# Chris10M/Ev2Hands

Measured on AMD Instinct MI355X. Metric: event-windows/sec at B=256 N=2048 (f16x2), higher is better.
Workload: dtype f32 (each f32 operand split into 2 fp16 planes with per-window power-of-two range scaling, 3 plane products per MAC on the f16 MFMA, f32 accumulate); 1 GPU; TEHNet.forward+MANO both hands, B=256/GPU N=2048 C=4 fp32, E-clouds, random-init 342-key checkpoint, synthetic MANO-shaped assets; global_batch=256, points=2048, channels=4, precision=f16x2, forwards_in_flight=1, world_size_seen=1, parallelism=batch-shard x1

## Files before the change

ev2hands_amd/csrc/points.hip:

```cpp
#include <cstdlib>
#include "common.hpp"
#include "ev2hands_hip.h"

namespace {

typedef float f32x2 __attribute__((ext_vector_type(2)));

__device__ __forceinline__ float sqnorm3(float x, float y, float z) {
    return __fadd_rn(__fadd_rn(__fmul_rn(x, x), __fmul_rn(y, y)), __fmul_rn(z, z));
}

__global__ __launch_bounds__(256) void prep_points_kernel(float* __restrict__ xyz_cm, int C, int N, int mhlnes,
                                                          float4* __restrict__ pts4, float4* __restrict__ feat8,
                                                          unsigned* __restrict__ amax) {
    const int b = blockIdx.y;
    const int n = blockIdx.x * 256 + threadIdx.x;
    float* base = xyz_cm + (size_t)b * C * N;
    float f[8];
#pragma unroll
    for (int c = 0; c < 8; ++c) f[c] = (c < C && n < N) ? base[(size_t)c * N + n] : 0.f;
    if (mhlnes && n < N) {
        float s = f[3];
        for (int c = 4; c < C; ++c) s = __fadd_rn(s, f[c]);
        s = s / (float)(C - 3);
        f[2] = s;
        base[(size_t)2 * N + n] = s;
    }
    if (amax) {
        unsigned m = 0u;
#pragma unroll
        for (int c = 0; c < 8; ++c) m = max(m, __float_as_uint(f[c]) & 0x7fffffffu);
        m = wave_max_u32_dpp(m);
        if ((threadIdx.x & 63) == 0 && m) atomicMax(&amax[b], m);
    }
    if (n >= N) return;
    pts4[(size_t)b * N + n] = make_float4(f[0], f[1], f[2], sqnorm3(f[0], f[1], f[2]));
    feat8[((size_t)b * N + n) * 2 + 0] = make_float4(f[0], f[1], f[2], f[3]);
    feat8[((size_t)b * N + n) * 2 + 1] = make_float4(f[4], f[5], f[6], f[7]);
}

struct FpsJobs {
    int njobs;
    int S[3];
    const int64_t* init[3];
    int32_t* idx[3];
    float4* ctr[3];
    int s_begin, s_end;
    float* state; int state_ld;
};

template <int PPT, int THREADS = 256, bool LDS_PTS = true>
__global__ __launch_bounds__(THREADS) void fps_kernel(const float4* __restrict__ pts4, int N, FpsJobs jobs) {
    extern __shared__ __attribute__((aligned(16))) char smem_raw[];
    float4* spts = reinterpret_cast<float4*>(smem_raw);
    constexpr int NW = THREADS / 64;
    __shared__ unsigned long long skey[2][NW];

    const int b = blockIdx.x;
    const int job = blockIdx.y;
    const int S = jobs.S[job];
    const int tid = threadIdx.x, lane = tid & 63, wave = tid >> 6;
    const float4* src = pts4 + (size_t)b * N;

    constexpr bool REG_PTS = !(PPT >= 32 && THREADS >= 1024);
    float px[REG_PTS ? PPT : 1], py[REG_PTS ? PPT : 1], pz[REG_PTS ? PPT : 1], md[PPT];
#pragma unroll
    for (int j = 0; j < PPT; ++j) {
        const int p = j * THREADS + tid;
        if constexpr (REG_PTS || LDS_PTS) {
            float4 v = (p < N) ? src[p] : make_float4(0.f, 0.f, 0.f, 0.f);
            if (LDS_PTS && p < N) spts[p] = v;
            if constexpr (REG_PTS) { px[j] = v.x; py[j] = v.y; pz[j] = v.z; }
        }
        md[j] = 1e10f;
    }
    __syncthreads();
    int tid_v = tid;
    auto coord = [&](int j, float& x, float& y, float& z) {
        if constexpr (REG_PTS) { x = px[j]; y = py[j]; z = pz[j]; }
        else {
            const unsigned pc = (unsigned)min(j * THREADS + tid_v, N - 1);
            const float4 v = *reinterpret_cast<const float4*>(reinterpret_cast<const char*>(src) + (size_t)pc * sizeof(float4));
            x = v.x; y = v.y; z = v.z;
        }
    };

    int far = (int)jobs.init[job][b];
    int32_t* oidx = jobs.idx[job] + (size_t)b * S;
    float4* octr = jobs.ctr[job] + (size_t)b * S;
    const int i_begin = min(jobs.s_begin, S), i_end = min(jobs.s_end, S);
    if (i_begin >= i_end) return;
    float* st = jobs.state ? jobs.state + ((size_t)b * jobs.njobs + job) * jobs.state_ld : nullptr;
    if (i_begin > 0) {
#pragma unroll
        for (int j = 0; j < PPT; ++j) md[j] = st[j * THREADS + tid];
        far = reinterpret_cast<const int*>(st)[jobs.state_ld - 4];
    }

    for (int i = i_begin; i < i_end; ++i) {
        if constexpr (!REG_PTS) asm volatile("" : "+v"(tid_v));
        const float4 c = LDS_PTS ? spts[far] : src[far];
        if (tid == 0) { oidx[i] = far; octr[i] = c; }
        unsigned long long best = 0ull;
        if constexpr (PPT >= 2) {
            const f32x2 cx = {c.x, c.x}, cy = {c.y, c.y}, cz = {c.z, c.z};
#pragma unroll
            for (int j = 0; j < PPT; j += 2) {
                float x0, y0, z0, x1, y1, z1;
                coord(j, x0, y0, z0);
                coord(j + 1, x1, y1, z1);
                const f32x2 dx = f32x2{x0, x1} - cx, dy = f32x2{y0, y1} - cy, dz = f32x2{z0, z1} - cz;
                const f32x2 d = (dx * dx + dy * dy) + dz * dz;
#pragma unroll
                for (int e = 0; e < 2; ++e) {
                    const int p = (j + e) * THREADS + tid;
                    if (d[e] < md[j + e]) md[j + e] = d[e];
                    const unsigned long long key =
                        ((unsigned long long)__float_as_uint(md[j + e]) << 32) | (unsigned long long)(0xffffffffu - (unsigned)p);
                    if (p < N && key > best) best = key;
                }
                if constexpr (!REG_PTS) {
                    if ((j & 6) == 6) __builtin_amdgcn_sched_barrier(0);
                }
            }
        } else {
#pragma unroll
            for (int j = 0; j < PPT; ++j) {
                const int p = j * THREADS + tid;
                float x0, y0, z0;
                coord(j, x0, y0, z0);
                const float dx = __fsub_rn(x0, c.x), dy = __fsub_rn(y0, c.y), dz = __fsub_rn(z0, c.z);
                const float d = sqnorm3(dx, dy, dz);
                if (d < md[j]) md[j] = d;
                const unsigned long long key =
                    ((unsigned long long)__float_as_uint(md[j]) << 32) | (unsigned long long)(0xffffffffu - (unsigned)p);
                if (p < N && key > best) best = key;
            }
        }
        best = wave_max_u64_dpp(best);
        if (lane == 0) skey[i & 1][wave] = best;
        __syncthreads();
        unsigned long long k0 = skey[i & 1][0];
#pragma unroll
        for (int w = 1; w < NW; ++w) { const unsigned long long kw = skey[i & 1][w]; k0 = k0 > kw ? k0 : kw; }
        far = (int)(0xffffffffu - (unsigned)(k0 & 0xffffffffull));
    }
    if (i_end < S) {
#pragma unroll
        for (int j = 0; j < PPT; ++j) st[j * THREADS + tid] = md[j];
        if (tid == 0) reinterpret_cast<int*>(st)[jobs.state_ld - 4] = far;
    }
}

struct BallArgs {
    int nrad;
    float r2[3];
    int K[3];
    int32_t* gidx[3];
    int32_t* cnt;
    int cpw;
    int nchunk;
    int s_off, s_cnt;
};

constexpr int BALL_CTR_PER_WG = 4, BALL_UNR = 4;

__global__ __launch_bounds__(256) void ball_query_kernel(const float4* __restrict__ pts4, const float4* __restrict__ ctr4,
                                                         int N, int S, BallArgs a) {
    const int L = xcd_remap(blockIdx.x, gridDim.x);
    const int b = L / a.nchunk;
    const int tid = threadIdx.x, lane = tid & 63, wave = tid >> 6;
    const float4* src = pts4 + (size_t)b * N;
    (void)tid;
    const int s_begin = a.s_off + (L - b * a.nchunk) * a.cpw;
    for (int s = s_begin + wave; s < s_begin + a.cpw && s < a.s_off + a.s_cnt; s += 4) {
        const float4 c = ctr4[(size_t)b * S + s];
        int cnt[3] = {0, 0, 0};
        int first[3] = {0, 0, 0};
        int32_t* gbase[3];
#pragma unroll
        for (int i = 0; i < 3; ++i) gbase[i] = (i < a.nrad) ? a.gidx[i] + ((size_t)b * S + s) * a.K[i] : nullptr;
        for (int base = 0; base < N; base += 64 * BALL_UNR) {
            float d[BALL_UNR];
#pragma unroll
            for (int u = 0; u < BALL_UNR; ++u) {
                const int p = base + 64 * u + lane;
                const float4 q = src[p < N ? p : N - 1];
                const float dot = __fmaf_rn(c.z, q.z, __fmaf_rn(c.y, q.y, __fmul_rn(c.x, q.x)));
                d[u] = __fadd_rn(__fadd_rn(__fmul_rn(-2.f, dot), c.w), q.w);
            }
            bool done = true;
#pragma unroll
            for (int i = 0; i < 3; ++i) {
                if (i < a.nrad && cnt[i] < a.K[i]) {
#pragma unroll
                    for (int u = 0; u < BALL_UNR; ++u) {
                        const int p = base + 64 * u + lane;
                        const bool in = (p < N) && !(d[u] > a.r2[i]);
                        const unsigned long long m = __ballot(in);
                        if (cnt[i] == 0 && m != 0ull) first[i] = base + 64 * u + __ffsll((long long)m) - 1;
                        const int pos = cnt[i] + (int)__builtin_amdgcn_mbcnt_hi((unsigned)(m >> 32), __builtin_amdgcn_mbcnt_lo((unsigned)m, 0u));
                        if (in && pos < a.K[i]) gbase[i][pos] = p;
                        cnt[i] += __popcll(m);
                    }
                    done = done && (cnt[i] >= a.K[i]);
                }
            }
            if (done) break;
        }
#pragma unroll
        for (int i = 0; i < 3; ++i) {
            if (i < a.nrad) {
                const int have = cnt[i] < a.K[i] ? cnt[i] : a.K[i];
                for (int pos = have + lane; pos < a.K[i]; pos += 64)
                    a.gidx[i][((size_t)b * S + s) * a.K[i] + pos] = first[i];
                if (a.cnt && lane == 0) a.cnt[((size_t)b * S + s) * a.nrad + i] = have;
            }
        }
    }
}

constexpr int NN_PTS_PER_WG = 256;
constexpr int NN_MAX_N2 = 4096;

__global__ __launch_bounds__(256) void three_nn_interp_kernel(const float4* __restrict__ pts1, const float4* __restrict__ pts2,
                                                              int N1, int N2, const float* __restrict__ feat2, int ldf2, int D,
                                                              float* __restrict__ out, int ldo,
                                                              int32_t* __restrict__ nn_idx, float* __restrict__ nn_w,
                                                              unsigned* __restrict__ amax, int ppw) {
    extern __shared__ __attribute__((aligned(16))) char smem_raw[];
    float4* s2 = reinterpret_cast<float4*>(smem_raw);
    int* sidx = reinterpret_cast<int*>(s2 + N2);
    float* sw = reinterpret_cast<float*>(sidx + NN_PTS_PER_WG * 3);
    const int b = blockIdx.y;
    const int tid = threadIdx.x, lane = tid & 63, wave = tid >> 6;
    for (int p = tid; p < N2; p += 256) s2[p] = pts2[(size_t)b * N2 + p];
    __syncthreads();

    const int n = blockIdx.x * ppw + tid;
    if (tid < ppw && n < N1) {
        const float4 q = pts1[(size_t)b * N1 + n];
        float d0 = INFINITY, d1 = INFINITY, d2 = INFINITY;
        int i0 = 0, i1 = 0, i2 = 0;
        for (int s = 0; s < N2; ++s) {
            const float4 c = s2[s];
            const float dot = __fmaf_rn(q.z, c.z, __fmaf_rn(q.y, c.y, __fmul_rn(q.x, c.x)));
            const float d = __fadd_rn(__fadd_rn(__fmul_rn(-2.f, dot), q.w), c.w);
            if (d < d2) {
                if (d < d1) {
                    d2 = d1; i2 = i1;
                    if (d < d0) { d1 = d0; i1 = i0; d0 = d; i0 = s; }
                    else        { d1 = d;  i1 = s; }
                } else { d2 = d; i2 = s; }
            }
        }
        const float r0 = __fdiv_rn(1.0f, __fadd_rn(d0, 1e-8f));
        const float r1 = __fdiv_rn(1.0f, __fadd_rn(d1, 1e-8f));
        const float r2 = __fdiv_rn(1.0f, __fadd_rn(d2, 1e-8f));
        const float norm = __fadd_rn(__fadd_rn(r0, r1), r2);
        const float w0 = __fdiv_rn(r0, norm), w1 = __fdiv_rn(r1, norm), w2 = __fdiv_rn(r2, norm);
        sidx[tid * 3 + 0] = i0; sidx[tid * 3 + 1] = i1; sidx[tid * 3 + 2] = i2;
        sw[tid * 3 + 0] = w0; sw[tid * 3 + 1] = w1; sw[tid * 3 + 2] = w2;
        if (nn_idx) {
            int32_t* o = nn_idx + ((size_t)b * N1 + n) * 3;
            o[0] = i0; o[1] = i1; o[2] = i2;
        }
        if (nn_w) {
            float* o = nn_w + ((size_t)b * N1 + n) * 3;
            o[0] = w0; o[1] = w1; o[2] = w2;
        }
    }
    __syncthreads();
    if (!out) return;
    const int D4 = D >> 2;
    float am = 0.f;
    const int pw = ppw >> 2;
#pragma unroll 1
    for (int t0 = wave * pw; t0 < wave * pw + pw; t0 += 4) {
        if (blockIdx.x * ppw + t0 >= N1) break;
        for (int c = lane; c < D4; c += 64) {
            float4 a[4], bq[4], cq[4];
            float w0[4], w1[4], w2[4];
#pragma unroll
            for (int u = 0; u < 4; ++u) {
                const int t = t0 + u;
                const int j0 = sidx[t * 3 + 0], j1 = sidx[t * 3 + 1], j2 = sidx[t * 3 + 2];
                w0[u] = sw[t * 3 + 0]; w1[u] = sw[t * 3 + 1]; w2[u] = sw[t * 3 + 2];
                const bool live = blockIdx.x * ppw + t < N1;
                a[u] = reinterpret_cast<const float4*>(feat2 + ((size_t)b * N2 + (live ? j0 : 0)) * ldf2)[c];
                bq[u] = reinterpret_cast<const float4*>(feat2 + ((size_t)b * N2 + (live ? j1 : 0)) * ldf2)[c];
                cq[u] = reinterpret_cast<const float4*>(feat2 + ((size_t)b * N2 + (live ? j2 : 0)) * ldf2)[c];
            }
#pragma unroll
            for (int u = 0; u < 4; ++u) {
                const int nn = blockIdx.x * ppw + t0 + u;
                if (nn >= N1) break;
                float4 r;
                r.x = __fadd_rn(__fadd_rn(__fmul_rn(a[u].x, w0[u]), __fmul_rn(bq[u].x, w1[u])), __fmul_rn(cq[u].x, w2[u]));
                r.y = __fadd_rn(__fadd_rn(__fmul_rn(a[u].y, w0[u]), __fmul_rn(bq[u].y, w1[u])), __fmul_rn(cq[u].y, w2[u]));
                r.z = __fadd_rn(__fadd_rn(__fmul_rn(a[u].z, w0[u]), __fmul_rn(bq[u].z, w1[u])), __fmul_rn(cq[u].z, w2[u]));
                r.w = __fadd_rn(__fadd_rn(__fmul_rn(a[u].w, w0[u]), __fmul_rn(bq[u].w, w1[u])), __fmul_rn(cq[u].w, w2[u]));
                reinterpret_cast<float4*>(out + ((size_t)b * N1 + nn) * ldo)[c] = r;
                am = fmaxf(fmaxf(am, fmaxf(fabsf(r.x), fabsf(r.y))), fmaxf(fabsf(r.z), fabsf(r.w)));
            }
        }
    }
    if (amax) {
        const unsigned m = wave_max_u32_dpp(__float_as_uint(am));
        if (lane == 0 && m) atomicMax(&amax[b], m);
    }
}

}

extern "C" int ev2h_prep_points(float* xyz_cm, int B, int C, int N, int mhlnes, float* pts4, float* feat8, uint32_t* amax,
                                ev2h_stream_t stream) {
    EV2H_CHECK_ARG(xyz_cm && pts4 && feat8);
    EV2H_CHECK_ARG(B > 0 && N > 0 && C >= 4 && C <= 8);
    dim3 grid(ceil_div(N, 256), B);
    prep_points_kernel<<<grid, 256, 0, (hipStream_t)stream>>>(xyz_cm, C, N, mhlnes, (float4*)pts4, (float4*)feat8, amax);
    EV2H_CHECK_LAUNCH();
    return EV2H_OK;
}

size_t ev2h_fps_state_ld(int N) {
    const int threads = N <= 2048 ? 256 : (N <= 8192 ? 512 : 1024);
    const int ppt = N <= 256 ? 1 : N <= 512 ? 2 : N <= 1024 ? 4 : N <= 2048 ? 8 : N <= 4096 ? 8 : N <= 8192 ? 16 : N <= 16384 ? 16 : 32;
    return (size_t)threads * ppt + 4;
}

int ev2h_fps_multi_chunk(const float* pts4, int B, int N, int njobs, const int* S, const int64_t* const* init, int32_t* const* idx, float* const* ctr4,
                         int s_begin, int s_end, float* state, ev2h_stream_t stream);

extern "C" int ev2h_fps_multi(const float* pts4, int B, int N, int njobs, const int* S, const int64_t* const* init,
                              int32_t* const* idx, float* const* ctr4, ev2h_stream_t stream) {
    return ev2h_fps_multi_chunk(pts4, B, N, njobs, S, init, idx, ctr4, 0, 0x7fffffff, nullptr, stream);
}

int ev2h_fps_multi_chunk(const float* pts4, int B, int N, int njobs, const int* S, const int64_t* const* init, int32_t* const* idx, float* const* ctr4,
                         int s_begin, int s_end, float* state, ev2h_stream_t stream) {
    EV2H_CHECK_ARG(pts4 && S && init && idx && ctr4);
    EV2H_CHECK_ARG(B > 0 && N > 0 && N <= 32768 && njobs >= 1 && njobs <= 3);
    EV2H_CHECK_ARG(s_begin >= 0 && s_end > s_begin);
    FpsJobs jobs{};
    jobs.njobs = njobs;
    jobs.s_begin = s_begin; jobs.s_end = s_end; jobs.state = state; jobs.state_ld = (int)ev2h_fps_state_ld(N);
    for (int j = 0; j < njobs; ++j) {
        EV2H_CHECK_ARG(S[j] > 0 && init[j] && idx[j] && ctr4[j]);
        jobs.S[j] = S[j];
        jobs.init[j] = init[j];
        jobs.idx[j] = idx[j];
        jobs.ctr[j] = (float4*)ctr4[j];
        EV2H_CHECK_ARG(state || (s_begin == 0 && s_end >= S[j]));
    }
    dim3 grid(B, njobs);
    const size_t lds = (size_t)N * sizeof(float4);
    hipStream_t st = (hipStream_t)stream;
    const float4* p = (const float4*)pts4;
    if (N > 2048 && N <= 8192) {
        static PerDevice attr_set{};
        EV2H_ONCE_PER_DEVICE(attr_set,
            EV2H_CHECK_HIP(hipFuncSetAttribute(reinterpret_cast<const void*>(fps_kernel<8, 512, true>),
                                               hipFuncAttributeMaxDynamicSharedMemorySize, 4096 * 16));
            EV2H_CHECK_HIP(hipFuncSetAttribute(reinterpret_cast<const void*>(fps_kernel<16, 512, true>),
                                               hipFuncAttributeMaxDynamicSharedMemorySize, 8192 * 16)););
    }
    if (N <= 256) fps_kernel<1><<<grid, 256, lds, st>>>(p, N, jobs);
    else if (N <= 512) fps_kernel<2><<<grid, 256, lds, st>>>(p, N, jobs);
    else if (N <= 1024) fps_kernel<4><<<grid, 256, lds, st>>>(p, N, jobs);
    else if (N <= 2048) fps_kernel<8><<<grid, 256, lds, st>>>(p, N, jobs);
    else if (N <= 4096) fps_kernel<8, 512, true><<<grid, 512, lds, st>>>(p, N, jobs);
    else if (N <= 8192) fps_kernel<16, 512, true><<<grid, 512, lds, st>>>(p, N, jobs);
    else if (N <= 16384) fps_kernel<16, 1024, false><<<grid, 1024, 0, st>>>(p, N, jobs);
    else fps_kernel<32, 1024, false><<<grid, 1024, 0, st>>>(p, N, jobs);
    EV2H_CHECK_LAUNCH();
    return EV2H_OK;
}

extern "C" int ev2h_fps(const float* pts4, int B, int N, int S, const int64_t* init, int32_t* idx, float* ctr4,
                        ev2h_stream_t stream) {
    return ev2h_fps_multi(pts4, B, N, 1, &S, &init, &idx, &ctr4, stream);
}

int ev2h_ball_query_range(const float* pts4, const float* ctr4, int B, int N, int S, int s_off, int s_cnt, int nrad, const double* radius,
                          const int* nsample, int32_t* const* gidx, int32_t* cnt, ev2h_stream_t stream);

extern "C" int ev2h_ball_query(const float* pts4, const float* ctr4, int B, int N, int S, int nrad, const double* radius,
                               const int* nsample, int32_t* const* gidx, int32_t* cnt, ev2h_stream_t stream) {
    return ev2h_ball_query_range(pts4, ctr4, B, N, S, 0, S, nrad, radius, nsample, gidx, cnt, stream);
}

int ev2h_ball_query_range(const float* pts4, const float* ctr4, int B, int N, int S, int s_off, int s_cnt, int nrad, const double* radius,
                          const int* nsample, int32_t* const* gidx, int32_t* cnt, ev2h_stream_t stream) {
    EV2H_CHECK_ARG(pts4 && ctr4 && radius && nsample && gidx);
    EV2H_CHECK_ARG(B > 0 && N > 0 && N <= 32768 && S > 0 && nrad >= 1 && nrad <= 3 && s_off >= 0 && s_cnt > 0 && s_off + s_cnt <= S);
    BallArgs a{};
    a.nrad = nrad;
    for (int i = 0; i < nrad; ++i) {
        EV2H_CHECK_ARG(gidx[i] && nsample[i] > 0);
        a.r2[i] = (float)(radius[i] * radius[i]);
        a.K[i] = nsample[i];
        a.gidx[i] = gidx[i];
    }
    a.cnt = cnt;
    a.cpw = BALL_CTR_PER_WG;
    a.s_off = s_off; a.s_cnt = s_cnt;
    a.nchunk = ceil_div(s_cnt, a.cpw);
    ball_query_kernel<<<dim3((unsigned)a.nchunk * (unsigned)B), 256, 0, (hipStream_t)stream>>>((const float4*)pts4, (const float4*)ctr4, N, S, a);
    EV2H_CHECK_LAUNCH();
    return EV2H_OK;
}

extern "C" int ev2h_three_nn_interp(const float* pts1_4, const float* pts2_4, int B, int N1, int N2, const float* feat2,
                                    int ldf2, int D, float* out, int ldo, int32_t* nn_idx, float* nn_w, uint32_t* out_amax,
                                    ev2h_stream_t stream) {
    EV2H_CHECK_ARG(pts1_4 && pts2_4);
    EV2H_CHECK_ARG(B > 0 && N1 > 0 && N2 >= 3 && N2 <= NN_MAX_N2);
    if (out) EV2H_CHECK_ARG(feat2 && D > 0 && (D % 4) == 0 && (ldf2 % 4) == 0 && (ldo % 4) == 0);
    const int ppw = ((long)ceil_div(N1, NN_PTS_PER_WG) * B < 128) ? 64 : NN_PTS_PER_WG;
    dim3 grid(ceil_div(N1, ppw), B);
    const size_t lds = (size_t)N2 * sizeof(float4) + NN_PTS_PER_WG * 3 * (sizeof(int) + sizeof(float));
    if (lds > 64 * 1024) {
        static PerDevice attr_set{};
        EV2H_ONCE_PER_DEVICE(attr_set,
            EV2H_CHECK_HIP(hipFuncSetAttribute(reinterpret_cast<const void*>(three_nn_interp_kernel), hipFuncAttributeMaxDynamicSharedMemorySize,
                                               NN_MAX_N2 * (int)sizeof(float4) + NN_PTS_PER_WG * 3 * (int)(sizeof(int) + sizeof(float)))););
    }
    three_nn_interp_kernel<<<grid, 256, lds, (hipStream_t)stream>>>((const float4*)pts1_4, (const float4*)pts2_4, N1, N2, feat2,
                                                                    ldf2, D, out, ldo, nn_idx, nn_w, out_amax, ppw);
    EV2H_CHECK_LAUNCH();
    return EV2H_OK;
}
```

Before: 22330 event-windows/s.

## Process multiple centers per wave in ball query with prefetched point loads

The ball query kernel is templated so each wave can handle up to four centers, reusing every loaded point tile across those centers instead of reloading it per center. The next tile is software-prefetched, and a combined ballot against the largest still-active radius skips the per-radius ballots when no lane is in range. The wide variant is chosen only when the grid would stay large, which trades fewer redundant point loads for more registers per wave and less parallelism per center.

```diff
diff --git a/ev2hands_amd/csrc/points.hip b/ev2hands_amd/csrc/points.hip
--- a/ev2hands_amd/csrc/points.hip
+++ b/ev2hands_amd/csrc/points.hip
@@ -163,58 +163,111 @@
     int s_off, s_cnt;
 };
 
-constexpr int BALL_CTR_PER_WG = 4, BALL_UNR = 4;
-
+constexpr int BALL_UNR = 4;
+constexpr int BALL_CPW_MAX = 4;
+
+template <int CPW>
 __global__ __launch_bounds__(256) void ball_query_kernel(const float4* __restrict__ pts4, const float4* __restrict__ ctr4,
                                                          int N, int S, BallArgs a) {
     const int L = xcd_remap(blockIdx.x, gridDim.x);
     const int b = L / a.nchunk;
-    const int tid = threadIdx.x, lane = tid & 63, wave = tid >> 6;
+    const int tid = threadIdx.x, lane = tid & 63, wave = __builtin_amdgcn_readfirstlane(tid >> 6);
     const float4* src = pts4 + (size_t)b * N;
-    (void)tid;
-    const int s_begin = a.s_off + (L - b * a.nchunk) * a.cpw;
-    for (int s = s_begin + wave; s < s_begin + a.cpw && s < a.s_off + a.s_cnt; s += 4) {
-        const float4 c = ctr4[(size_t)b * S + s];
-        int cnt[3] = {0, 0, 0};
-        int first[3] = {0, 0, 0};
-        int32_t* gbase[3];
-#pragma unroll
-        for (int i = 0; i < 3; ++i) gbase[i] = (i < a.nrad) ? a.gidx[i] + ((size_t)b * S + s) * a.K[i] : nullptr;
-        for (int base = 0; base < N; base += 64 * BALL_UNR) {
+    const int s0 = a.s_off + (L - b * a.nchunk) * a.cpw + wave * CPW;
+    const int ncen = min(CPW, a.s_off + a.s_cnt - s0);
+    if (ncen <= 0) return;
+    const size_t row0 = (size_t)b * S + s0;
+    float4 c[CPW];
+    int cnt[CPW][3], first[CPW][3];
+#pragma unroll
+    for (int j = 0; j < CPW; ++j) {
+        c[j] = ctr4[row0 + (j < ncen ? j : 0)];
+        if constexpr (CPW > 1) asm volatile("" : "+v"(c[j].x), "+v"(c[j].y), "+v"(c[j].z), "+v"(c[j].w));
+#pragma unroll
+        for (int i = 0; i < 3; ++i) cnt[j][i] = first[j][i] = 0;
+    }
+    int K[3];
+    unsigned r2b[3];
+#pragma unroll
+    for (int i = 0; i < 3; ++i) {
+        K[i] = __builtin_amdgcn_readfirstlane(a.K[i]);
+        r2b[i] = (unsigned)__builtin_amdgcn_readfirstlane((int)__float_as_uint(a.r2[i]));
+    }
+    auto live = [&](int j) { return j < ncen && (cnt[j][0] < K[0] || cnt[j][1] < K[1] || cnt[j][2] < K[2]); };
+    const unsigned off_last = (unsigned)(N - 1) * (unsigned)sizeof(float4);
+    unsigned off[BALL_UNR];
+    float4 q[BALL_UNR], qn[BALL_UNR];
+#pragma unroll
+    for (int u = 0; u < BALL_UNR; ++u) off[u] = (unsigned)(64 * u + lane) * (unsigned)sizeof(float4);
+    auto load_step = [&]() {
+#pragma unroll
+        for (int u = 0; u < BALL_UNR; ++u) {
+            qn[u] = *reinterpret_cast<const float4*>(reinterpret_cast<const char*>(src) + (size_t)min(off[u], off_last));
+            off[u] += 64 * BALL_UNR * (unsigned)sizeof(float4);
+        }
+    };
+    load_step();
+    for (int base = 0; base < N; base += 64 * BALL_UNR) {
+#pragma unroll
+        for (int u = 0; u < BALL_UNR; ++u) q[u] = qn[u];
+        load_step();
+        unsigned long long vm[BALL_UNR] = {~0ull, ~0ull, ~0ull, ~0ull};
+        if (base + 64 * BALL_UNR > N) {
+#pragma unroll
+            for (int u = 0; u < BALL_UNR; ++u) {
+                const int left = N - base - 64 * u;
+                vm[u] = left >= 64 ? ~0ull : left <= 0 ? 0ull : (1ull << left) - 1ull;
+            }
+        }
+        bool any_live = false;
+#pragma unroll
+        for (int j = 0; j < CPW; ++j) {
+            if (!live(j)) continue;
             float d[BALL_UNR];
 #pragma unroll
             for (int u = 0; u < BALL_UNR; ++u) {
-                const int p = base + 64 * u + lane;
-                const float4 q = src[p < N ? p : N - 1];
-                const float dot = __fmaf_rn(c.z, q.z, __fmaf_rn(c.y, q.y, __fmul_rn(c.x, q.x)));
-                d[u] = __fadd_rn(__fadd_rn(__fmul_rn(-2.f, dot), c.w), q.w);
-            }
-            bool done = true;
-#pragma unroll
-            for (int i = 0; i < 3; ++i) {
-                if (i < a.nrad && cnt[i] < a.K[i]) {
-#pragma unroll
-                    for (int u = 0; u < BALL_UNR; ++u) {
-                        const int p = base + 64 * u + lane;
-                        const bool in = (p < N) && !(d[u] > a.r2[i]);
-                        const unsigned long long m = __ballot(in);
-                        if (cnt[i] == 0 && m != 0ull) first[i] = base + 64 * u + __ffsll((long long)m) - 1;
-                        const int pos = cnt[i] + (int)__builtin_amdgcn_mbcnt_hi((unsigned)(m >> 32), __builtin_amdgcn_mbcnt_lo((unsigned)m, 0u));
-                        if (in && pos < a.K[i]) gbase[i][pos] = p;
-                        cnt[i] += __popcll(m);
+                const float dot = __fmaf_rn(c[j].z, q[u].z, __fmaf_rn(c[j].y, q[u].y, __fmul_rn(c[j].x, q[u].x)));
+                d[u] = __fadd_rn(__fadd_rn(__fmul_rn(-2.f, dot), c[j].w), q[u].w);
+            }
+            unsigned rtop_bits = 0u;
+#pragma unroll
+            for (int i = 0; i < 3; ++i) rtop_bits = max(rtop_bits, r2b[i] & (0u - (unsigned)(cnt[j][i] < K[i])));
+            const float rtop = __uint_as_float(rtop_bits);
+            unsigned long long mtop[BALL_UNR];
+#pragma unroll
+            for (int u = 0; u < BALL_UNR; ++u) mtop[u] = __builtin_amdgcn_ballot_w64(!(d[u] > rtop)) & vm[u];
+            if ((mtop[0] | mtop[1] | mtop[2] | mtop[3]) != 0ull) {
+#pragma unroll
+                for (int u = 0; u < BALL_UNR; ++u) {
+                    if (mtop[u] == 0ull) continue;
+                    const int p = base + 64 * u + lane;
+#pragma unroll
+                    for (int i = 0; i < 3; ++i) {
+                        if (cnt[j][i] < K[i]) {
+                            const unsigned long long m = __builtin_amdgcn_ballot_w64(!(d[u] > a.r2[i])) & vm[u];
+                            if (m == 0ull) continue;
+                            if (cnt[j][i] == 0) first[j][i] = base + 64 * u + __ffsll((long long)m) - 1;
+                            const int pos = cnt[j][i] + (int)__builtin_amdgcn_mbcnt_hi((unsigned)(m >> 32), __builtin_amdgcn_mbcnt_lo((unsigned)m, 0u));
+                            if (!(d[u] > a.r2[i]) && p < N && pos < K[i]) a.gidx[i][(row0 + j) * a.K[i] + pos] = p;
+                            cnt[j][i] = __builtin_amdgcn_readfirstlane(cnt[j][i] + __popcll(m));
+                        }
                     }
-                    done = done && (cnt[i] >= a.K[i]);
                 }
             }
-            if (done) break;
-        }
+            any_live = any_live || live(j);
+        }
+        if (!any_live) break;
+    }
+#pragma unroll
+    for (int j = 0; j < CPW; ++j) {
+        if (j >= ncen) break;
 #pragma unroll
         for (int i = 0; i < 3; ++i) {
             if (i < a.nrad) {
-                const int have = cnt[i] < a.K[i] ? cnt[i] : a.K[i];
+                const int have = cnt[j][i] < a.K[i] ? cnt[j][i] : a.K[i];
                 for (int pos = have + lane; pos < a.K[i]; pos += 64)
-                    a.gidx[i][((size_t)b * S + s) * a.K[i] + pos] = first[i];
-                if (a.cnt && lane == 0) a.cnt[((size_t)b * S + s) * a.nrad + i] = have;
+                    a.gidx[i][(row0 + j) * a.K[i] + pos] = first[j][i];
+                if (a.cnt && lane == 0) a.cnt[(row0 + j) * a.nrad + i] = have;
             }
         }
     }
@@ -403,10 +456,13 @@
         a.gidx[i] = gidx[i];
     }
     a.cnt = cnt;
-    a.cpw = BALL_CTR_PER_WG;
     a.s_off = s_off; a.s_cnt = s_cnt;
+    const bool wide = (long)ceil_div(s_cnt, 4 * BALL_CPW_MAX) * B >= 4096;
+    a.cpw = wide ? 4 * BALL_CPW_MAX : 4;
     a.nchunk = ceil_div(s_cnt, a.cpw);
-    ball_query_kernel<<<dim3((unsigned)a.nchunk * (unsigned)B), 256, 0, (hipStream_t)stream>>>((const float4*)pts4, (const float4*)ctr4, N, S, a);
+    const dim3 grid((unsigned)a.nchunk * (unsigned)B);
+    if (wide) ball_query_kernel<BALL_CPW_MAX><<<grid, 256, 0, (hipStream_t)stream>>>((const float4*)pts4, (const float4*)ctr4, N, S, a);
+    else ball_query_kernel<1><<<grid, 256, 0, (hipStream_t)stream>>>((const float4*)pts4, (const float4*)ctr4, N, S, a);
     EV2H_CHECK_LAUNCH();
     return EV2H_OK;
 }
```

Measured after the change: 22530 event-windows/s, median of 6. Within noise of the previous version (+0.9%).
